# GiviMAD/rustpotter

Hardware: AMD Instinct MI355X
Metric: 10ms-frame MFCC+DTW scorings/sec (higher is better)
Workload: dtype f32; 1 GPU; C3: 65536 synthetic 16 kHz f32 streams x 8 templates per GPU (4 s streams, L=100, K=5, band 5, ScoreMode::Max, avg gate off); streams_per_gpu=65536, templates=8, template_chunks=1, device=AMD Radeon Graphics, compute_units=256, build=gfx950, world_size=1, backend=none (one rank)

## Files before the change

### rustpotter_amd/csrc/rp_dtw_mfma.hip

```cpp
#include "rp_device.h"

#include <cstdlib>

namespace rp {

namespace {

typedef unsigned u32x6 __attribute__((ext_vector_type(6)));

constexpr int kMK = 5;
constexpr int kMWin = 32;
constexpr int mfma_slots(int nt) { return nt == 8 ? 12 : 16; }
constexpr int mfma_tiles(int nt) { return nt == 8 ? 3 : 2; }
constexpr int kMSlotsMax = 16;
constexpr int mfma_acc_reg(int nt, int slot, int p, int e) {
    return nt == 8 ? 4 * (slot % 4) + 2 * p + e : 4 * ((slot % 8) >> 1) + 2 * (slot & 1) + e;
}

#ifdef RP_MFMA_CVT_BACK
typedef __fp16 fp16x2 __attribute__((ext_vector_type(2)));
__device__ __forceinline__ float lo_f32(unsigned p) { return (float)__builtin_bit_cast(fp16x2, p)[0]; }
__device__ __forceinline__ float hi_f32(unsigned p) { return (float)__builtin_bit_cast(fp16x2, p)[1]; }
#endif

template <int W, int NT>
__host__ __device__ constexpr int mfma_last_use(int u, int g) {
    int last = -1;
    for (int q = 0; q < 2 * W; ++q)
        if (((u + q + mfma_slots(NT) - W + 2) % mfma_slots(NT)) / (32 / NT) == g) last = q;
    return last;
}

}

#ifdef RP_MFMA_TRACE
#define RP_TRACE(slot)                                                                                                        \
    do {                                                                                                                      \
        if ((threadIdx.x & 63) == 0 && ((threadIdx.x >> 6) == 0 || (threadIdx.x >> 6) == NW - 1) && blockIdx.x < 96)             \
            reinterpret_cast<unsigned long long *>(sched + 1024)[(blockIdx.x * 2 + ((threadIdx.x >> 6) ? 1 : 0)) * 8 + (slot)] = \
                __builtin_amdgcn_s_memrealtime();                                                                             \
    } while (0)
#else
#define RP_TRACE(slot)
#endif

#ifndef RP_MFMA_WAVES_PER_EU
#define RP_MFMA_WAVES_PER_EU 0
#endif
#if RP_MFMA_WAVES_PER_EU
#define RP_MFMA_OCC __attribute__((amdgpu_waves_per_eu(RP_MFMA_WAVES_PER_EU, RP_MFMA_WAVES_PER_EU)))
#else
#define RP_MFMA_OCC
#endif
template <int W, int NW, bool GX, int NT, bool P3>
RP_MFMA_OCC __global__ __launch_bounds__(64 * NW, 1) void dtw_mfma_kernel(
    const float *__restrict__ mfcc, size_t frame_pitch, size_t n_frames_total, size_t total_tiles, unsigned n_chunks, int chunk_base,
    size_t first_win, size_t n_win, size_t out_win_pitch, const DtwChunk *__restrict__ chunks, const uint4 *__restrict__ aimg, int T,
    float score_ref, float *__restrict__ scores, float *__restrict__ avg, size_t n_streams, int max_len, const uint32_t *__restrict__ list,
    const uint32_t *__restrict__ count, uint32_t dense_min, float abandon_nc, uint32_t *__restrict__ sched, unsigned static_rounds,
    float *__restrict__ agg_out, uint32_t *__restrict__ agg_hot, float agg_threshold, uint32_t *__restrict__ fix) {
    constexpr int K = kMK, B = 2 * W, NS = mfma_slots(NT), NTILE = mfma_tiles(NT), SPT = 32 / NT, NP = NT / 4;
    constexpr int kRowBytes = P3 ? kDtwMfma3RowBytes : kDtwMfmaRowBytes;
#ifndef RP_MFMA_GX_PD
    constexpr int PD = GX ? (NS % 3 == 0 ? 3 : 4) : 1;
#else
    constexpr int PD = GX ? RP_MFMA_GX_PD : 1;
#endif
    static_assert(NS % PD == 0, "the frame ring's slot must be a compile-time index");
    static_assert(NT == 8 || NT == 4, "template slots per chunk");
    static_assert(B + 2 <= NS, "the band and its two neighbours must fit the circular row slots");
    size_t total_entries = n_streams * n_win;
    if (list) {
        const uint32_t n_listed = *count;
        if (dense_min && n_listed >= dense_min) return;
        total_entries = n_listed;
        total_tiles = ((size_t)n_listed + kMWin - 1) / kMWin;
    } else if (count && *count < dense_min) return;
    extern __shared__ __attribute__((aligned(16))) unsigned char smem[];
    RP_TRACE(0);
    const unsigned ci = blockIdx.x % n_chunks;
    const unsigned n_groups = gridDim.x / n_chunks;
    const DtwChunk *ch = chunks + chunk_base + ci;
    const int L = ch->len;
    const int a_bytes = (max_len + kMSlotsMax) * kRowBytes;
    const int xs_floats = dtw_mfma_stage_floats(max_len);
    const int tid = threadIdx.x, lane = tid & 63, wave = tid >> 6;
    dtw_load_aimg<64 * NW>(smem, aimg, P3 ? ch->aimg3_off : ch->aimg_off, (L + kMSlotsMax) * kRowBytes / 16, tid);
    __syncthreads();
    RP_TRACE(1);
    float *xs = reinterpret_cast<float *>(smem + a_bytes) + wave * xs_floats;
    (void)xs;
    const int n = lane & 31, h = lane >> 5;
    const int mrow = lane & 31;
    const int jj = NT == 8 ? mrow >> 3 : 2 * (mrow >> 3) + ((mrow >> 1) & 1);
    const int tA = NT == 8 ? ((mrow >> 2) & 1) * 4 + (mrow & 3) : ((mrow >> 2) & 1) * 2 + (mrow & 1);
    const unsigned a_lane = (unsigned)(h * 128 + tA * 16);
    unsigned dl[SPT];
#pragma unroll
    for (int e = 0; e < SPT; ++e) dl[e] = (unsigned)(((e - jj + NS) % NS) * kRowBytes);
    const unsigned sel_one = h ? 0x07060100u : 0x03020100u;
    const unsigned sel_c2 = h ? 0x03020706u : 0x07060302u;
    const unsigned mask_c2 = h ? 0xffff0000u : 0u;
    (void)sel_c2; (void)mask_c2;
    const float abandon_cost = abandon_nc * (float)(L + L);
    bool slot_real[2 * NP], slot_avg[2 * NP];
#pragma unroll
    for (int e = 0; e < 2 * NP; ++e) {
        slot_real[e] = 2 * NP * h + e < ch->count;
        slot_avg[e] = slot_real[e] && ch->tid[2 * NP * h + e] >= T;
    }

    uint32_t *next_tile = sched + 2 * (chunk_base + ci);
    unsigned round = 0;
    const size_t chunk_waves = (size_t)n_groups * NW;
    for (;;) {
        const size_t tile = dtw_next_tile<NW>(next_tile, round, static_rounds, chunk_waves, n_chunks, wave, lane);
        if (tile >= total_tiles) break;
        const size_t f0 = tile * kMWin;
        bool valid;
        size_t s;
        int w;
        const float *xw;
        if (GX) {
            size_t f = f0 + n;
            valid = f < total_entries;
            if (list) f = list[valid ? f : total_entries - 1];
            s = valid ? f / n_win : 0;
            w = valid ? (int)(f - s * n_win) : 0;
            xw = mfcc + (s * frame_pitch + first_win + (size_t)w) * K;
        } else {
            const size_t sA = f0 / n_win;
            const int wA = (int)(f0 - sA * n_win);
            const int nA = (int)n_win - wA < kMWin ? (int)n_win - wA : kMWin;
            const int nB = (nA < kMWin && sA + 1 < n_streams) ? kMWin - nA : 0;
            const int segA = nA + L + 3;
            auto stage =[&](const float *src, size_t g0, int n_floats, float *dst) {
                for (int i0 = lane; i0 < n_floats; i0 += 256) {
                    float v[4];
#pragma unroll
                    for (int j = 0; j < 4; ++j) {
                        const int i = i0 + 64 * j;
                        v[j] = (i < n_floats && g0 + (size_t)(i / K) < n_frames_total) ? src[g0 * K + i] : 0.f;
                    }
#pragma unroll
                    for (int j = 0; j < 4; ++j)
                        if (i0 + 64 * j < n_floats) dst[i0 + 64 * j] = v[j];
                }
            };
            stage(mfcc + sA * frame_pitch * K, first_win + wA, segA * K, xs);
            if (nB > 0) stage(mfcc + (sA + 1) * frame_pitch * K, first_win, (nB + L + 3) * K, xs + segA * K);
            wave_lds_sync();
            const bool inA = n < nA;
            valid = inA || (n - nA < nB);
            s = inA ? sA : sA + 1;
            w = inA ? wA + n : n - nA;
            xw = xs + (inA ? n : (valid ? segA + n - nA : 0)) * K;
        }
        const float *xa = xw + (h ? 3 : 0);
        const float *x2 = xw + 2;
        float mua = 0.f, mub = 0.f, mu2 = 0.f;
#ifndef RP_MFMA_GX_MEAN_UNROLL
#define RP_MFMA_GX_MEAN_UNROLL 20
#endif
#ifndef RP_MFMA_MEAN_UNROLL
#define RP_MFMA_MEAN_UNROLL 8
#endif
        constexpr int kMeanUnroll = GX ? RP_MFMA_GX_MEAN_UNROLL : RP_MFMA_MEAN_UNROLL;
#pragma unroll kMeanUnroll
        for (int i = 0; i < L; ++i) { mua += xa[i * K]; mub += xa[i * K + 1]; mu2 += x2[i * K]; }
        mua = mua / (float)L; mub = mub / (float)L; mu2 = mu2 / (float)L;
        if (round == 1) RP_TRACE(2);

        v2f Q[NP][B + 1];
#pragma unroll
        for (int p = 0; p < NP; ++p) {
#pragma unroll
            for (int q = 0; q <= B; ++q) Q[p][q] = (v2f){RP_INF, RP_INF};
            Q[p][W - 1] = (v2f){0.f, 0.f};
        }
        u32x4 Areg[NTILE], Areg2[P3 ? NTILE : 1];
#pragma unroll
        for (int g = 0; g < NTILE; ++g) {
            const int slot = SPT * g + jj;
            int r = W - ((W - slot + NS) % NS);
            r = r < 1 ? 1 : r;
            Areg[g] = *reinterpret_cast<const u32x4 *>(smem + a_lane + (unsigned)(r - 1) * kRowBytes);
            if (P3) Areg2[g] = *reinterpret_cast<const u32x4 *>(smem + a_lane + 256u + (unsigned)(r - 1) * kRowBytes);
        }
        v16f acc[NTILE];
        u32x4 bop[2];
        u32x6 bv[P3 ? 2 : 1];
        (void)bv;

#define RP_P0(cc, rs) fa_[rs] = xa[((cc) - 1) * K]; fb_[rs] = xa[((cc) - 1) * K + 1]; f2_[rs] = x2[((cc) - 1) * K];
#define RP_P1(cc, rs) da_ = fa_[rs] - mua; db_ = fb_[rs] - mub; d2_ = f2_[rs] - mu2;
#define RP_P2(cc) own_ = fmaf(da_, da_, db_ * db_);
#define RP_P3(cc) { const auto sw_ = __builtin_amdgcn_permlane32_swap(__float_as_uint(own_), __float_as_uint(own_), false, false); \
                    bb_ = fmaf(d2_, d2_, __uint_as_float(sw_[0]) + __uint_as_float(sw_[1])); }
#define RP_P4(cc) inv_ = bb_ > 0.f ? __builtin_amdgcn_rsqf(bb_) : 0.f;
#define RP_P5(cc) ua_ = da_ * inv_; ub_ = db_ * inv_; u2_ = d2_ * inv_;
#define RP_HI2(hi, lo) __builtin_amdgcn_perm(__float_as_uint(hi), __float_as_uint(lo), 0x07060302u)
#define RP_AND(x, m) __uint_as_float(__float_as_uint(x) & (m))
#define RP_BSET(par, i, v) bv[par][i] = (v)
#define RP_P6(cc, par) if (P3) { x0a_ = RP_AND(ua_, 0xffff0000u); x0b_ = RP_AND(ub_, 0xffff0000u); x0c_ = RP_AND(u2_, 0xffff0000u); RP_BSET(par, 2, RP_HI2(ub_, ua_)); } \
                       else { bop[par].x = pkrtz(ua_, ub_); bop[par].z = bop[par].x; }
#ifndef RP_MFMA_CVT_BACK
#define RP_X0F(x, packed, hi) x0f(x)
#else
#define RP_X0F(x, packed, hi) ((hi) ? hi_f32(packed) : lo_f32(packed))
#endif
#define RP_P7(cc, par) if (P3) { r1a_ = ua_ - x0a_; r1b_ = ub_ - x0b_; r1c_ = u2_ - x0c_; RP_BSET(par, 3, RP_HI2(r1b_, r1a_)); } \
                       else { bop[par].y = pk_f16_second(ua_ - RP_X0F(ua_, bop[par].x, 0), ub_ - RP_X0F(ub_, bop[par].x, 1)); }
#ifndef RP_AB_NO_RANGE_TEST
#define RP_P8(cc) chk_ = fmaxf(fmaxf(chk_, inv_), bb_);   \
                  if (P3) { x1a_ = RP_AND(r1a_, 0xffff0000u); x1b_ = RP_AND(r1b_, 0xffff0000u); tc_ = RP_AND(r1c_, mask_c2); }
#else
#define RP_P8(cc) if (P3) { x1a_ = RP_AND(r1a_, 0xffff0000u); x1b_ = RP_AND(r1b_, 0xffff0000u); tc_ = RP_AND(r1c_, mask_c2); }
#endif
#define RP_P9(cc, par) if (P3) { RP_BSET(par, 0, RP_HI2(r1b_ - x1b_, r1a_ - x1a_)); RP_BSET(par, 1, __builtin_amdgcn_perm(__float_as_uint(r1c_ - tc_), __float_as_uint(u2_), sel_c2)); } \
                       else { const float x0_ = RP_X0F(u2_, pkrtz(u2_, 0.f), 0);  \
                         bop[par].w = __builtin_amdgcn_perm(0x3c000000u, pk_f16_second(x0_, u2_ - x0_), sel_one); }
#define RP_P10(cc, par) if (P3) { bv[par][4] = bv[par][2]; bv[par][5] = h ? 0x00003f80u : bv[par][1]; }
#define RP_PREP_ALL(cc, par) RP_P0(cc, (cc) % PD) RP_P1(cc, (cc) % PD) RP_P2(cc) RP_P3(cc) RP_P4(cc) RP_P5(cc) RP_P6(cc, par) RP_P7(cc, par) RP_P8(cc) RP_P9(cc, par) RP_P10(cc, par)
#define RP_AREF(cc, uu, GUARD)                                                                                                \
    {                                                                                                                         \
        const int sn = ((uu) + 1 + W) % NS, g = sn / SPT, e = sn % SPT;                                                       \
        int off = ((cc) + W - 1) * kRowBytes - (int)dl[e];                                                                    \
        if (GUARD) off = off < 0 ? 0 : off;                                                                                   \
        Areg[g] = *reinterpret_cast<const u32x4 *>(smem + a_lane + (unsigned)off);                                            \
        if (P3) Areg2[g] = *reinterpret_cast<const u32x4 *>(smem + a_lane + 256u + (unsigned)off);                            \
    }
#define RP_B1(par) __builtin_shufflevector(bv[P3 ? (par) : 0], bv[P3 ? (par) : 0], 0, 1, 2, 3)
#define RP_B2(par) __builtin_shufflevector(bv[P3 ? (par) : 0], bv[P3 ? (par) : 0], 2, 3, 4, 5)
#define RP_MFMA(g, par)                                                                                                       \
    do {                                                                                                                      \
        const v16f zero16 = {0.f, 0.f, 0.f, 0.f, 0.f, 0.f, 0.f, 0.f, 0.f, 0.f, 0.f, 0.f, 0.f, 0.f, 0.f, 0.f};                  \
        if (P3) acc[g] = __builtin_amdgcn_mfma_f32_32x32x16_bf16(__builtin_bit_cast(bf16x8, Areg[g]), __builtin_bit_cast(bf16x8, RP_B1(par)), zero16, 0, 0, 0); \
        else acc[g] = __builtin_amdgcn_mfma_f32_32x32x16_f16(__builtin_bit_cast(f16x8, Areg[g]), __builtin_bit_cast(f16x8, bop[par]), zero16, 0, 0, 0); \
    } while (0)
#define RP_MFMA2(g, par)                                                                                                      \
    do {                                                                                                                      \
        if (P3) acc[g] = __builtin_amdgcn_mfma_f32_32x32x16_bf16(__builtin_bit_cast(bf16x8, Areg2[g]), __builtin_bit_cast(bf16x8, RP_B2(par)), acc[g], 0, 0, 0); \
    } while (0)

#ifndef RP_P3_GAP
#define RP_P3_GAP 1
#endif
#define RP_STEP(GUARD)                                                                                                        \
    do {                                                                                                                      \
        RP_AREF(c + 1, (u + 1) % NS, GUARD)                                                                                   \
        v2f up[2] = {(v2f){RP_INF, RP_INF}, (v2f){RP_INF, RP_INF}};                                                           \
        _Pragma("unroll") for (int q = 0; q < B; ++q) {                                                                       \
            const int sl = (u + q + NS - W + 2) % NS;                                                                         \
            _Pragma("unroll") for (int p = 0; p < NP; ++p) {                 \
                const v2f cost = (v2f){acc[sl / SPT][mfma_acc_reg(NT, sl, p, 0)], acc[sl / SPT][mfma_acc_reg(NT, sl, p, 1)]}; \
                v2f m, v;                                                                                                     \
                m.x = fminf(fminf(up[p].x, Q[p][q + 1].x), Q[p][q].x);                                                        \
                m.y = fminf(fminf(up[p].y, Q[p][q + 1].y), Q[p][q].y);                                                        \
                v.x = cost.x + m.x; v.y = cost.y + m.y;  \
                if (GUARD) v = (c - W + 1 + q >= 1) ? v : (v2f){RP_INF, RP_INF};                                              \
                Q[p][q] = v;                                                                                                  \
                up[p] = v;                                                                                                    \
            }                                                                                                                 \
                                                                                              \
            if (!P3) {                                                                                                        \
            if (q == (0 * B) / 10) { RP_P1(c + 2, (u + 3) % PD) RP_P0(c + 2 + PD, (u + 3) % PD) } if (q == (2 * B) / 10) { RP_P2(c + 2) }                       \
            if (q == (3 * B) / 10) { RP_P3(c + 2) } if (q == (4 * B) / 10) { RP_P4(c + 2) } if (q == (5 * B) / 10) { RP_P5(c + 2) } \
            if (q == (6 * B) / 10) { RP_P6(c + 2, (u + 1) & 1) } if (q == (7 * B) / 10) { RP_P7(c + 2, (u + 1) & 1) }         \
            if (q == (8 * B) / 10) { RP_P8(c + 2) } if (q == (9 * B) / 10) { RP_P9(c + 2, (u + 1) & 1) }                      \
            } else {                             \
            if (q == (0 * B) / 11) { RP_P1(c + 2, (u + 3) % PD) RP_P0(c + 2 + PD, (u + 3) % PD) } if (q == (1 * B) / 11) { RP_P2(c + 2) }                       \
            if (q == (2 * B) / 11) { RP_P3(c + 2) } if (q == (3 * B) / 11) { RP_P4(c + 2) } if (q == (4 * B) / 11) { RP_P5(c + 2) } \
            if (q == (5 * B) / 11) { RP_P6(c + 2, (u + 1) & 1) } if (q == (6 * B) / 11) { RP_P7(c + 2, (u + 1) & 1) }         \
            if (q == (7 * B) / 11) { RP_P8(c + 2) } if (q == (8 * B) / 11) { RP_P9(c + 2, (u + 1) & 1) }                      \
            if (q == (9 * B) / 11) { RP_P10(c + 2, (u + 1) & 1) }                                                             \
            }                                                                                                                 \
            _Pragma("unroll") for (int g = 0; g < NTILE; ++g) {                                                               \
                if (mfma_last_use<W, NT>(u, g) == q) RP_MFMA(g, u & 1);                                                       \
                if (q >= RP_P3_GAP && mfma_last_use<W, NT>(u, g) == q - RP_P3_GAP) RP_MFMA2(g, u & 1);                        \
            }                                                                                                                 \
            __builtin_amdgcn_sched_barrier(0);                                                                                \
        }                                                                                                                     \
        _Pragma("unroll") for (int g = 0; g < NTILE; ++g) {                                                                   \
            if (mfma_last_use<W, NT>(u, g) < 0) { RP_MFMA(g, u & 1); RP_MFMA2(g, u & 1); }                                    \
            else if (RP_P3_GAP > 0 && mfma_last_use<W, NT>(u, g) > B - 1 - RP_P3_GAP) RP_MFMA2(g, u & 1);                     \
        }                                                                                                                     \
    } while (0)

        float fa_[PD], fb_[PD], f2_[PD], da_, db_, d2_, own_, bb_, inv_, ua_, ub_, u2_, chk_ = 0.f;
        float x0a_ = 0.f, x0b_ = 0.f, x0c_ = 0.f, r1a_ = 0.f, r1b_ = 0.f, r1c_ = 0.f, x1a_ = 0.f, x1b_ = 0.f, tc_ = 0.f;
        (void)x0a_; (void)x0b_; (void)x0c_; (void)r1a_; (void)r1b_; (void)r1c_; (void)x1a_; (void)x1b_; (void)tc_;
        RP_AREF(1, 0, true)
        RP_PREP_ALL(1, 1)
        RP_MFMA(0, 1); RP_MFMA(1, 1);
        if (NTILE > 2) RP_MFMA(NTILE - 1, 1);
        RP_MFMA2(0, 1); RP_MFMA2(1, 1);
        if (NTILE > 2) RP_MFMA2(NTILE - 1, 1);
        RP_PREP_ALL(2, 0)
#pragma unroll
        for (int a = 0; a < PD; ++a) { RP_P0(3 + a, (3 + a) % PD) }
        __builtin_amdgcn_sched_barrier(0);
        int c0 = 1;
        bool dead = false;
        {
#pragma unroll
            for (int u = 0; u < NS; ++u) { const int c = c0 + u; RP_STEP(true); }
        }
#ifdef RP_MFMA_PRICE_NO_ABANDON
#define RP_ABANDON_ON false
#else
#define RP_ABANDON_ON (abandon_nc < RP_INF)
#endif
#define RP_ABANDON_CHECK()                                                                                                    \
    if (RP_ABANDON_ON) {                                                                                                \
        bool alive = false;                                                                                                   \
        _Pragma("unroll") for (int p = 0; p < NP; ++p) {                                                                      \
            v2f m = Q[p][0];                                                                                                  \
            _Pragma("unroll") for (int q = 1; q < B; ++q) m = (v2f){fminf(m.x, Q[p][q].x), fminf(m.y, Q[p][q].y)};             \
            alive = alive || (slot_real[2 * p] && (m.x <= abandon_cost || slot_avg[2 * p])) ||                                \
                    (slot_real[2 * p + 1] && (m.y <= abandon_cost || slot_avg[2 * p + 1]));                                   \
        }                                                                                                                     \
        if (!__any(alive && valid)) dead = true;                                                                              \
    }
        for (c0 = 1 + NS; c0 + NS - 1 <= L; c0 += NS) {
            RP_ABANDON_CHECK()
            if (dead) break;
#pragma unroll
            for (int u = 0; u < NS; ++u) { const int c = c0 + u; RP_STEP(false); }
        }
        if (!dead && c0 <= L) {
            RP_ABANDON_CHECK()
            if (!dead) {
#pragma unroll
                for (int u = 0; u < NS - 1; ++u) {
                    const int c = c0 + u;
                    if (c <= L) RP_STEP(false);
                }
            }
        }
#undef RP_ABANDON_CHECK
#undef RP_ABANDON_ON
#undef RP_STEP
#undef RP_MFMA
#undef RP_MFMA2
#undef RP_P10
#undef RP_HI2
#undef RP_AND
#undef RP_BSET
#undef RP_B1
#undef RP_B2
#undef RP_AREF
#undef RP_PREP_ALL
#undef RP_P0
#undef RP_P1
#undef RP_P2
#undef RP_P3
#undef RP_P4
#undef RP_P5
#undef RP_P6
#undef RP_P7
#undef RP_P8
#undef RP_P9
#undef RP_X0F

        if (round == 1) RP_TRACE(3);
        float best = 0.f;
        if (valid) {
            const size_t row = s * out_win_pitch + (size_t)w;
            const float denom = (float)(L + L);
#pragma unroll
            for (int p = 0; p < NP; ++p) {
#pragma unroll
                for (int e = 0; e < 2; ++e) {
                    const int slot = 2 * NP * h + 2 * p + e;
                    if (slot < ch->count) {
                        const float cost = e ? Q[p][W - 2].y : Q[p][W - 2].x;
                        const float nc = cost / denom;
                        const float sc = dead ? 0.f : dtw_logistic(nc, score_ref);
                        const int t = ch->tid[slot];
                        if (t < T) { scores[row * T + t] = sc; best = fmaxf(best, sc); }
                        else if (!dead) avg[row] = sc;
                    }
                }
            }
            if (h == 0 && chk_ > kDtwFixLimit) dtw_fix_append(fix, row, (uint32_t)(chunk_base + (int)ci));
        }
        if (agg_out) {
            const auto sw_ = __builtin_amdgcn_permlane32_swap(__float_as_uint(best), __float_as_uint(best), false, false);
            const float m = fmaxf(__uint_as_float(sw_[0]), __uint_as_float(sw_[1]));
            if (valid && h == 0) {
                agg_out[s * out_win_pitch + (size_t)w] = m;
                if (agg_hot && m > agg_threshold) agg_hot[s] = 1u;
            }
        }
        if (!GX) wave_lds_sync();
        if (round == 1) RP_TRACE(4);
    }
    RP_TRACE(5);
    __syncthreads();
    RP_TRACE(6);
    dtw_release_tiles(next_tile, n_groups, tid);
}

bool dtw_mfma_supported(const TemplatesDev &t, int band, size_t n_win, bool from_global, int slots, float score_ref) {
    const int mode = t.arith_mode();
    if (mode == kArithStrictF32 || t.K != kMK || !(mode == kArithFastSplit ? t.aimg : t.aimg3) || t.max_diff != 0) return false;
    const bool p3 = mode != kArithFastSplit;
    if (!p3 && !(score_ref >= kDtwMfmaMinScoreRef)) return false;
    if (slots == 8 ? (band < 3 || band > 5) : band != 5) return false;
    if (!from_global && n_win < (size_t)kMWin) return false;
    if (slots == 8 ? t.mfma_min_len < mfma_slots(8) : t.mfma_min_len4 < mfma_slots(4)) return false;
    return dtw_mfma_lds_bytes(t.max_len, 8, p3 ? kDtwMfma3RowBytes : kDtwMfmaRowBytes) <= 160 * 1024;
}

hipError_t launch_dtw_mfma(const DtwCall &c, int slots, int chunk_base, int n_chunks, bool from_global, const GateList &gate) {
    const TemplatesDev &t = *c.t;
    const DtwWork &wk = c.wk;
    const DtwFusedAgg *fuse = gate.fuse;
    if (n_chunks <= 0 || c.S == 0 || c.n_win == 0) return hipSuccess;
    const bool p3 = t.arith_mode() != kArithFastSplit;
    dtw_mark(wk, kDtwRanMfma | (p3 ? kDtwRanBf16x3 : kDtwRanF16x2));
    if (fuse && (n_chunks != 1 || gate.list || gate.count)) return hipErrorInvalidValue;
    float *agg_out = fuse ? fuse->agg : nullptr;
    uint32_t *agg_hot = fuse ? fuse->hot : nullptr;
    const float agg_threshold = fuse ? fuse->threshold : 0.f;
    if (gate.list && !from_global) return hipErrorNotSupported;
    const size_t total_tiles = (c.S * c.n_win + kMWin - 1) / kMWin;
    const int row_bytes = p3 ? kDtwMfma3RowBytes : kDtwMfmaRowBytes;
    int nw = dtw_mfma_lds_bytes(t.max_len, 12, row_bytes) <= 160 * 1024 ? 12 : 8;
    if (p3 && slots == 8) {
        static const int env_nw = [] { const char *e = std::getenv("RP_MFMA3_WAVES"); return e ? std::atoi(e) : 0; }();
        if (env_nw != 12) nw = 8;
    }
    const size_t lds = dtw_mfma_lds_bytes(t.max_len, nw, row_bytes);
    const void *image = p3 ? t.aimg3 : t.aimg;
    if (!wk.sched || !wk.fix) return hipErrorInvalidValue;
    unsigned blocks, static_rounds;
    if (hipError_t e = mfma_grid(total_tiles, n_chunks, nw, gate.list != nullptr, blocks, static_rounds); e != hipSuccess) return e;
#define RP_LAUNCH_MFMA_P(WW, NW, GXV, NT, PP)                                                                                       \
    do {                                                                                                                            \
        if (hipError_t e = allow_dynamic_lds(reinterpret_cast<const void *>(dtw_mfma_kernel<WW, NW, GXV, NT, PP>), 160 * 1024); e != hipSuccess) return e; \
        hipLaunchKernelGGL((dtw_mfma_kernel<WW, NW, GXV, NT, PP>), dim3(blocks), dim3(64 * NW), lds, c.st, c.mfcc, c.frame_pitch, c.frame_pitch, \
                           total_tiles, (unsigned)n_chunks, chunk_base, c.first_win, c.n_win, c.out_win_pitch, t.chunks,             \
                           reinterpret_cast<const uint4 *>(image), t.T, c.score_ref, c.scores, c.avg, c.S, t.max_len, gate.list, gate.count, \
                           gate.dense_min, gate.abandon_nc, wk.sched, static_rounds, agg_out, agg_hot, agg_threshold, wk.fix);      \
    } while (0)
#define RP_LAUNCH_MFMA(WW, NW, GXV, NT)                                                                                             \
    do {                                                                                                                            \
        if (p3) RP_LAUNCH_MFMA_P(WW, NW, GXV, NT, true); else RP_LAUNCH_MFMA_P(WW, NW, GXV, NT, false);                             \
    } while (0)
#define RP_LAUNCH_MFMA_W(WW, NT)                                                                                                    \
    do {                                                                                                                            \
        if (from_global) { if (nw == 12) RP_LAUNCH_MFMA(WW, 12, true, NT); else RP_LAUNCH_MFMA(WW, 8, true, NT); }                  \
        else { if (nw == 12) RP_LAUNCH_MFMA(WW, 12, false, NT); else RP_LAUNCH_MFMA(WW, 8, false, NT); }                            \
    } while (0)
    if (slots == 4) {
        if (c.band != 5) return hipErrorNotSupported;
        RP_LAUNCH_MFMA_W(5, 4);
    } else {
        switch (c.band) {
        case 3: RP_LAUNCH_MFMA_W(3, 8); break;
        case 4: RP_LAUNCH_MFMA_W(4, 8); break;
        case 5: RP_LAUNCH_MFMA_W(5, 8); break;
        default: return hipErrorNotSupported;
        }
    }
#undef RP_LAUNCH_MFMA_W
#undef RP_LAUNCH_MFMA
#undef RP_LAUNCH_MFMA_P
    return hipGetLastError();
}

}
```

Baseline: 885.8 million scorings/s.

## Prepare whole frame per lane and exchange halves via permlane32 swap in P3 MFMA DTW

For the P3 (three-term split) path, except the GX NW=12 NT=8 config, each lane now centres, normalises and splits all five coefficients of one frame (lanes h=0/1 handle consecutive frames). The packed B operands for two frames are then exchanged between wave halves with permlane32_swap, instead of each half preparing its own coefficient subset for every frame. Means are shared across the halves with the same swap, and the range-check maximum is merged at the end. The goal is to remove duplicated per-frame prep work spread across the DTW step. The cost is more registers, extra cross-lane swaps, and a new tail-guard path for the range check.

```diff
diff --git a/rustpotter_amd/csrc/rp_dtw_mfma.hip b/rustpotter_amd/csrc/rp_dtw_mfma.hip
--- a/rustpotter_amd/csrc/rp_dtw_mfma.hip
+++ b/rustpotter_amd/csrc/rp_dtw_mfma.hip
@@ -30,6 +30,8 @@
         if (((u + q + mfma_slots(NT) - W + 2) % mfma_slots(NT)) / (32 / NT) == g) last = q;
     return last;
 }
+
+constexpr bool mfma_whole_frame(int nw, bool gx, int nt, bool p3) { return p3 && !(gx && nw == 12 && nt == 8); }
 
 }
 
@@ -67,6 +69,9 @@
     constexpr int PD = GX ? RP_MFMA_GX_PD : 1;
 #endif
     static_assert(NS % PD == 0, "the frame ring's slot must be a compile-time index");
+    constexpr bool WF = mfma_whole_frame(NW, GX, NT, P3);
+    constexpr int PP = GX ? 2 : 1;
+    static_assert(NS % (2 * PP) == 0, "the pair ring's slot must be a compile-time index");
     static_assert(NT == 8 || NT == 4, "template slots per chunk");
     static_assert(B + 2 <= NS, "the band and its two neighbours must fit the circular row slots");
     size_t total_entries = n_streams * n_win;
@@ -169,6 +174,17 @@
 #pragma unroll kMeanUnroll
         for (int i = 0; i < L; ++i) { mua += xa[i * K]; mub += xa[i * K + 1]; mu2 += x2[i * K]; }
         mua = mua / (float)L; mub = mub / (float)L; mu2 = mu2 / (float)L;
+        float mu_[K] = {0.f, 0.f, 0.f, 0.f, 0.f};
+        (void)mu_;
+        if (WF) {
+            const auto sa_ = __builtin_amdgcn_permlane32_swap(__float_as_uint(mua), __float_as_uint(mua), false, false);
+            const auto sb_ = __builtin_amdgcn_permlane32_swap(__float_as_uint(mub), __float_as_uint(mub), false, false);
+            mu_[0] = __uint_as_float(sa_[0]); mu_[3] = __uint_as_float(sa_[1]);
+            mu_[1] = __uint_as_float(sb_[0]); mu_[4] = __uint_as_float(sb_[1]);
+            mu_[2] = mu2;
+        }
+        const float *xh = xw + h * K;
+        (void)xh;
         if (round == 1) RP_TRACE(2);
 
         v2f Q[NP][B + 1];
@@ -222,6 +238,38 @@
                          bop[par].w = __builtin_amdgcn_perm(0x3c000000u, pk_f16_second(x0_, u2_ - x0_), sel_one); }
 #define RP_P10(cc, par) if (P3) { bv[par][4] = bv[par][2]; bv[par][5] = h ? 0x00003f80u : bv[par][1]; }
 #define RP_PREP_ALL(cc, par) RP_P0(cc, (cc) % PD) RP_P1(cc, (cc) % PD) RP_P2(cc) RP_P3(cc) RP_P4(cc) RP_P5(cc) RP_P6(cc, par) RP_P7(cc, par) RP_P8(cc) RP_P9(cc, par) RP_P10(cc, par)
+#define RP_W_LOAD(cc, rs) g_[rs][0] = xh[((cc) - 1) * K]; g_[rs][1] = xh[((cc) - 1) * K + 1]; g_[rs][2] = xh[((cc) - 1) * K + 2];                 \
+                          g_[rs][3] = xh[((cc) - 1) * K + 3]; g_[rs][4] = xh[((cc) - 1) * K + 4];
+#define RP_W_NEAR(cc, rs) if (!GX) { RP_W_LOAD(cc, rs) }
+#define RP_W_CENTRE(cc, rs) d_[0] = g_[rs][0] - mu_[0]; d_[1] = g_[rs][1] - mu_[1]; d_[2] = g_[rs][2] - mu_[2]; d_[3] = g_[rs][3] - mu_[3];         \
+                            d_[4] = g_[rs][4] - mu_[4]; if (GX) { RP_W_LOAD((cc) + 2 * PP, rs) }
+#define RP_W_NORM() bb_ = fmaf(d_[2], d_[2], fmaf(d_[0], d_[0], d_[1] * d_[1]) + fmaf(d_[3], d_[3], d_[4] * d_[4]));
+#define RP_W_SCALE() w_[0] = d_[0] * inv_; w_[1] = d_[1] * inv_; w_[2] = d_[2] * inv_; w_[3] = d_[3] * inv_; w_[4] = d_[4] * inv_;
+#ifndef RP_AB_NO_RANGE_TEST
+#define RP_W_CHK(in_window) if (in_window) chk_ = fmaxf(fmaxf(chk_, inv_), bb_);
+#else
+#define RP_W_CHK(in_window)
+#endif
+#define RP_W_X0() x0_[0] = RP_AND(w_[0], 0xffff0000u); x0_[1] = RP_AND(w_[1], 0xffff0000u); x0_[2] = RP_AND(w_[2], 0xffff0000u);         \
+                  x0_[3] = RP_AND(w_[3], 0xffff0000u); x0_[4] = RP_AND(w_[4], 0xffff0000u);                                              \
+                  lo_[2] = RP_HI2(w_[1], w_[0]); up_[2] = RP_HI2(w_[4], w_[3]);
+#define RP_W_R1() r_[0] = w_[0] - x0_[0]; r_[1] = w_[1] - x0_[1]; r_[2] = w_[2] - x0_[2]; r_[3] = w_[3] - x0_[3]; r_[4] = w_[4] - x0_[4]; \
+                  lo_[3] = RP_HI2(r_[1], r_[0]); up_[3] = RP_HI2(r_[4], r_[3]); lo_[1] = RP_HI2(r_[2], w_[2]);
+#define RP_W_X1() y_[0] = RP_AND(r_[0], 0xffff0000u); y_[1] = RP_AND(r_[1], 0xffff0000u); y_[2] = RP_AND(r_[2], 0xffff0000u);            \
+                  y_[3] = RP_AND(r_[3], 0xffff0000u); y_[4] = RP_AND(r_[4], 0xffff0000u);
+#define RP_W_X2() lo_[0] = RP_HI2(r_[1] - y_[1], r_[0] - y_[0]); up_[0] = RP_HI2(r_[4] - y_[4], r_[3] - y_[3]);                          \
+                  up_[1] = __builtin_amdgcn_perm(__float_as_uint(r_[2] - y_[2]), __float_as_uint(w_[2]), 0x03020706u);
+#define RP_W_SWAP()                                                                                                           \
+    {                                                                                                                         \
+        _Pragma("unroll") for (int i = 0; i < 4; ++i) {                                                                       \
+            const auto sw_ = __builtin_amdgcn_permlane32_swap(lo_[i], up_[i], false, false);                                  \
+            bv[1][i] = sw_[0]; bv[0][i] = sw_[1];                                                                             \
+        }                                                                                                                     \
+        bv[1][4] = bv[1][2]; bv[1][5] = h ? 0x00003f80u : bv[1][1];                                                           \
+        bv[0][4] = bv[0][2]; bv[0][5] = h ? 0x00003f80u : bv[0][1];                                                           \
+    }
+#define RP_W_FIRST(cc, rs) RP_W_NEAR(cc, rs) RP_W_CENTRE(cc, rs) RP_W_NORM() RP_P4(cc) RP_W_SCALE()
+#define RP_W_SECOND(in_window) RP_W_CHK(in_window) RP_W_X0() RP_W_R1() RP_W_X1() RP_W_X2()
 #define RP_AREF(cc, uu, GUARD)                                                                                                \
     {                                                                                                                         \
         const int sn = ((uu) + 1 + W) % NS, g = sn / SPT, e = sn % SPT;                                                       \
@@ -246,7 +294,7 @@
 #ifndef RP_P3_GAP
 #define RP_P3_GAP 1
 #endif
-#define RP_STEP(GUARD)                                                                                                        \
+#define RP_STEP(GUARD, TAIL)                                                                                                      \
     do {                                                                                                                      \
         RP_AREF(c + 1, (u + 1) % NS, GUARD)                                                                                   \
         v2f up[2] = {(v2f){RP_INF, RP_INF}, (v2f){RP_INF, RP_INF}};                                                           \
@@ -263,7 +311,15 @@
                 up[p] = v;                                                                                                    \
             }                                                                                                                 \
                                                                                               \
-            if (!P3) {                                                                                                        \
+            if (WF) {   \
+            const int gi = (u & 1) ? q : B + q;                                                                              \
+            if (gi == 0) { RP_W_SWAP() RP_W_NEAR(c + 3, ((u + 3) / 2) % PP) }                                                 \
+            if (gi == (1 * 2 * B) / 9) { RP_W_CENTRE(c + 3, ((u + 3) / 2) % PP) }                                             \
+            if (gi == (2 * 2 * B) / 9) { RP_W_NORM() } if (gi == (3 * 2 * B) / 9) { RP_P4(c + 3) } if (gi == (4 * 2 * B) / 9) { RP_W_SCALE() } \
+             \
+            if (gi == (5 * 2 * B) / 9) { RP_W_CHK(!(TAIL) || c + h <= L) RP_W_X0() } if (gi == (6 * 2 * B) / 9) { RP_W_R1() }  \
+            if (gi == (7 * 2 * B) / 9) { RP_W_X1() } if (gi == (8 * 2 * B) / 9) { RP_W_X2() }                                 \
+            } else if (!P3) {                                                                                                 \
             if (q == (0 * B) / 10) { RP_P1(c + 2, (u + 3) % PD) RP_P0(c + 2 + PD, (u + 3) % PD) } if (q == (2 * B) / 10) { RP_P2(c + 2) }                       \
             if (q == (3 * B) / 10) { RP_P3(c + 2) } if (q == (4 * B) / 10) { RP_P4(c + 2) } if (q == (5 * B) / 10) { RP_P5(c + 2) } \
             if (q == (6 * B) / 10) { RP_P6(c + 2, (u + 1) & 1) } if (q == (7 * B) / 10) { RP_P7(c + 2, (u + 1) & 1) }         \
@@ -290,21 +346,31 @@
         float fa_[PD], fb_[PD], f2_[PD], da_, db_, d2_, own_, bb_, inv_, ua_, ub_, u2_, chk_ = 0.f;
         float x0a_ = 0.f, x0b_ = 0.f, x0c_ = 0.f, r1a_ = 0.f, r1b_ = 0.f, r1c_ = 0.f, x1a_ = 0.f, x1b_ = 0.f, tc_ = 0.f;
         (void)x0a_; (void)x0b_; (void)x0c_; (void)r1a_; (void)r1b_; (void)r1c_; (void)x1a_; (void)x1b_; (void)tc_;
+        float g_[PP][K], d_[K], w_[K], x0_[K], r_[K], y_[K];
+        unsigned lo_[4], up_[4];
+        (void)g_; (void)d_; (void)w_; (void)x0_; (void)r_; (void)y_; (void)lo_; (void)up_; (void)da_; (void)db_; (void)d2_; (void)own_; (void)ua_; (void)ub_; (void)u2_;
         RP_AREF(1, 0, true)
-        RP_PREP_ALL(1, 1)
+        if (WF) {
+            if (GX) { RP_W_LOAD(1, 0) RP_W_LOAD(3, 1 % PP) }
+            RP_W_FIRST(1, 0) RP_W_SECOND(true) RP_W_SWAP()
+        }
+        else { RP_PREP_ALL(1, 1) }
         RP_MFMA(0, 1); RP_MFMA(1, 1);
         if (NTILE > 2) RP_MFMA(NTILE - 1, 1);
         RP_MFMA2(0, 1); RP_MFMA2(1, 1);
         if (NTILE > 2) RP_MFMA2(NTILE - 1, 1);
-        RP_PREP_ALL(2, 0)
-#pragma unroll
-        for (int a = 0; a < PD; ++a) { RP_P0(3 + a, (3 + a) % PD) }
+        if (WF) { RP_W_FIRST(3, 1 % PP) }
+        else {
+            RP_PREP_ALL(2, 0)
+#pragma unroll
+            for (int a = 0; a < PD; ++a) { RP_P0(3 + a, (3 + a) % PD) }
+        }
         __builtin_amdgcn_sched_barrier(0);
         int c0 = 1;
         bool dead = false;
         {
 #pragma unroll
-            for (int u = 0; u < NS; ++u) { const int c = c0 + u; RP_STEP(true); }
+            for (int u = 0; u < NS; ++u) { const int c = c0 + u; RP_STEP(true, false); }
         }
 #ifdef RP_MFMA_PRICE_NO_ABANDON
 #define RP_ABANDON_ON false
@@ -326,7 +392,7 @@
             RP_ABANDON_CHECK()
             if (dead) break;
 #pragma unroll
-            for (int u = 0; u < NS; ++u) { const int c = c0 + u; RP_STEP(false); }
+            for (int u = 0; u < NS; ++u) { const int c = c0 + u; RP_STEP(false, false); }
         }
         if (!dead && c0 <= L) {
             RP_ABANDON_CHECK()
@@ -334,7 +400,7 @@
 #pragma unroll
                 for (int u = 0; u < NS - 1; ++u) {
                     const int c = c0 + u;
-                    if (c <= L) RP_STEP(false);
+                    if (c <= L) RP_STEP(false, true);
                 }
             }
         }
@@ -344,6 +410,19 @@
 #undef RP_MFMA
 #undef RP_MFMA2
 #undef RP_P10
+#undef RP_W_LOAD
+#undef RP_W_NEAR
+#undef RP_W_CENTRE
+#undef RP_W_NORM
+#undef RP_W_SCALE
+#undef RP_W_CHK
+#undef RP_W_X0
+#undef RP_W_R1
+#undef RP_W_X1
+#undef RP_W_X2
+#undef RP_W_SWAP
+#undef RP_W_FIRST
+#undef RP_W_SECOND
 #undef RP_HI2
 #undef RP_AND
 #undef RP_BSET
@@ -364,6 +443,10 @@
 #undef RP_X0F
 
         if (round == 1) RP_TRACE(3);
+        if (WF) {
+            const auto sw_ = __builtin_amdgcn_permlane32_swap(__float_as_uint(chk_), __float_as_uint(chk_), false, false);
+            chk_ = fmaxf(__uint_as_float(sw_[0]), __uint_as_float(sw_[1]));
+        }
         float best = 0.f;
         if (valid) {
             const size_t row = s * out_win_pitch + (size_t)w;
```

Measured after the change: 904.3 million scorings/s (median of 6 runs). +2.1%, better.
